# illini-robomaster/irmv_detection

Hardware: AMD Instinct MI355X
Metric: end-to-end FPS (preprocess→NMS→PnP) 640×640 YOLOv8n, 1/2/4/8 MI355X (higher is better)
Workload: dtype f16

## Files before the change

### irmv_detection_amd/csrc/irmv_common.hpp

```cpp
#pragma once

#include <hip/hip_runtime.h>

#include <cstdint>
#include <cstdlib>

namespace irmv {

typedef _Float16 half_t;
typedef _Float16 half8 __attribute__((ext_vector_type(8)));
typedef _Float16 half4 __attribute__((ext_vector_type(4)));
typedef float f32x4 __attribute__((ext_vector_type(4)));

constexpr float kActScale = 1.44269504088896341f;
constexpr float kActUnscale = 0.693147180559945309f;
typedef unsigned int u32x4_t __attribute__((ext_vector_type(4)));
__device__ __forceinline__ float silu_rcp(float y) { return __builtin_amdgcn_rcpf(1.0f + __builtin_amdgcn_exp2f(-y)); }
__device__ __forceinline__ unsigned int silu_pack2(float y0, float y1)
{
    const float r0 = silu_rcp(y0), r1 = silu_rcp(y1);
    unsigned int o;
    asm("v_fma_mixlo_f16 %0, %1, %2, 0" : "=v"(o) : "v"(y0), "v"(r0));
    asm("v_fma_mixhi_f16 %0, %1, %2, 0" : "+v"(o) : "v"(y1), "v"(r1));
    return o;
}
__device__ __forceinline__ half8 silu_pack8(float y0, float y1, float y2, float y3, float y4, float y5, float y6, float y7)
{
    return __builtin_bit_cast(half8, (u32x4_t){silu_pack2(y0, y1), silu_pack2(y2, y3), silu_pack2(y4, y5), silu_pack2(y6, y7)});
}
__device__ __forceinline__ half4 silu_pack4(float y0, float y1, float y2, float y3)
{
    typedef unsigned int u32x2_t __attribute__((ext_vector_type(2)));
    return __builtin_bit_cast(half4, (u32x2_t){silu_pack2(y0, y1), silu_pack2(y2, y3)});
}
__device__ __forceinline__ void mfma_operand_fence(half4 &x) { asm volatile("s_nop 1" : "+v"(x)); }
__device__ __forceinline__ void mfma_operand_fence(half8 &x, half8 &y) { asm volatile("s_nop 1" : "+v"(x), "+v"(y)); }
__device__ __forceinline__ half_t silu_add_res(float y, float res)
{
    float p = y * silu_rcp(y);
    asm("" : "+v"(p));
    float s = p + res;
    asm("" : "+v"(s));
    return (half_t)s;
}

__device__ __forceinline__ void tile_image(int id, int tiles, int batch, int xcd, int &tile, int &image)
{
    const int full = xcd ? (batch >> 3) * 8 * tiles : 0;
    if (id < full) {
        const int j = id >> 3;
        image = (j / tiles) * 8 + (id & 7);
        tile = j % tiles;
    } else {
        const int r = id - full;
        image = (full / tiles) + r / tiles;
        tile = r % tiles;
    }
}

inline int xcd_image_order()
{
    const char *v = getenv("IRMV_XCD_IMAGES");
    return (v && v[0] == '0') ? 0 : 1;
}

inline int wres_stagger()
{
    const char *v = getenv("IRMV_WRES_STAGGER");
    return (v && v[0] == '0') ? 0 : 1;
}

constexpr int kHeadRec = 96;
constexpr int kClsOff = 64;
constexpr int kKptOff = 80;
constexpr int kCandCap = 8192;
constexpr int kMaxDetCap = 256;

struct AxisTap { int32_t i0, i1, w1, pad; };

struct PreArgs {
    const uint8_t *src;
    half_t *dst;
    const AxisTap *tx, *ty;
    int sw, sh, net, swap_rb;
    size_t src_slot_bytes;
};
void launch_preprocess(const PreArgs &a, int batch, hipStream_t s);
void launch_rotate180(const uint8_t *src, uint8_t *dst, int sw, int sh, hipStream_t s);
void launch_upload_frames(const uint8_t *src_host_mapped, uint8_t *dst, size_t bytes, int blocks, hipStream_t s);

constexpr int kBayerBandRows = 8;
struct BayerArgs {
    const uint8_t *raw;
    uint8_t *dst;
    size_t raw_slot_bytes, dst_slot_bytes;
    int W, H;
    int ry, rx;
    uint32_t gain[3];
};
void launch_demosaic(const BayerArgs &a, int batch, hipStream_t s);

struct Conv0Args {
    const half_t *x;
    half_t *y;
    const half_t *w;
    const float *b;
    int net, batch;
};
void launch_conv0(const Conv0Args &a, hipStream_t s);

constexpr int kFrontTileY = 4, kFrontTileX = 16;
constexpr int kFrontTileYDirect = 8;
constexpr int kFrontStageMax = 128 * 1024;
struct FrontArgs {
    const uint8_t *src;
    size_t src_slot_bytes;
    const AxisTap *tx, *ty;
    int vx0, vx1, vy0, vy1;
    int sw, sh, net, swap_rb;
    int fastx, fx_i0, fx_step;
    const half_t *w0;
    const float *b0;
    const half_t *w1;
    const float *b1;
    half_t *out;
    int out_ld;
    int tiles_x, tiles_y;
    int tile_y;
    int stage_bytes;
};
int front_min_stage_bytes(int tile_y = kFrontTileY);
bool front_prepare();
bool launch_front(const FrontArgs &a, int batch, hipStream_t s);

constexpr int kC2fTile = 16;
struct C2fArgs {
    const half_t *x;
    int x_ld;
    half_t *out;
    int out_ld;
    int S, tiles;
    const half_t *w_cv1, *w_m1, *w_m2, *w_cv2;
    const float *b_cv1, *b_m1, *b_m2, *b_cv2;
};
void launch_c2f2(const C2fArgs &a, int batch, hipStream_t s);

struct DwArgs {
    const half_t *x;
    int x_ld;
    half_t *y;
    int y_ld;
    const half_t *w;
    const float *b;
    int Hin, Win, Hout, Wout, C, stride;
};
void launch_dwconv3x3(const DwArgs &a, int batch, hipStream_t s);
struct ShufArgs {
    const half_t *a, *b;
    int a_ld, b_ld;
    half_t *out;
    int out_ld, bc;
    size_t pixels;
};
void launch_shuffle_cat(const ShufArgs &a, hipStream_t s);

struct ConvSeg {
    const half_t *p;
    int ld;
    int C;
    int shift;
};

constexpr int kC2f32TileH = 8, kC2f32TileW = 16;
struct C2f32Args {
    ConvSeg s0, s1;
    int cin1;
    half_t *cat;
    int cat_ld, prev_coff;
    half_t *out;
    int out_ld;
    int H, W, tiles_x, tiles_y;
    const half_t *w_cv1, *w_m1, *w_m2, *w_cv2;
    const float *b_cv1, *b_m1, *b_m2, *b_cv2;
};
size_t c2f32_lds_bytes(int mode);
bool launch_c2f32(int mode, bool shortcut, const C2f32Args &a, int batch, hipStream_t s);

constexpr int kBneckTile = 8;
struct BneckArgs {
    const half_t *yin;
    int yin_ld;
    half_t *ynext;
    int ynext_ld;
    const half_t *cat;
    int cat_ld;
    half_t *out;
    int out_ld;
    int H, W, tiles_x, tiles_y;
    const half_t *w_m1, *w_m2;
    const float *b_m1, *b_m2;
    const half_t *w_cv2;
    const float *b_cv2;
};
size_t bneck64_lds_bytes(int mode, int ks2);
bool launch_bneck64(int mode, int ks2, bool shortcut, const BneckArgs &a, int batch, hipStream_t s);

constexpr int kKpt3Tile = 10;
struct Kpt3Args {
    const half_t *x;
    int x_ld;
    int H, W, tiles_x, tiles_y;
    const half_t *w1;
    const float *b1;
    const half_t *w2;
    const float *b2;
    const half_t *w3;
    const float *b3;
    float *out;
    int out_ld;
};
bool kpt3_eligible(int cin);
bool launch_kpt3(const Kpt3Args &a, int cin, int batch, hipStream_t s);

struct ConvArgs {
    ConvSeg s0, s1;
    int Hin, Win;
    int Hout, Wout;
    int M;
    int Cin;
    const half_t *w;
    const float *bias;
    void *out;
    int out_ld;
    const half_t *res;
    int res_ld;
    int cout_pad;
    int ksteps;
    int pair;
    const half_t *w2;
    const float *bias2;
    float *out2;
    int out2_ld, n2;
    unsigned long long *scan_keys;
    int *scan_counts;
    float scan_thr;
    int scan_nc, scan_abase, scan_key_cap;
};

constexpr int kMultiMax = 6;
struct LdsMember {
    ConvArgs a;
    const half_t *wl;
    int tiles_x, tiles_y, twc_log2, patch_bytes, batch, tile2d;
    int gx, gy;
};
struct LdsMultiArgs {
    int n;
    int start[kMultiMax + 1];
    LdsMember m[kMultiMax];
};
struct DirectMultiArgs {
    int n;
    int start[kMultiMax + 1], gx[kMultiMax], gy[kMultiMax];
    ConvArgs a[kMultiMax];
};

struct ConvCfg {
    int ks, stride, mt, nt; bool cin16; int act; bool out_f32; bool lds; int ipw;
    bool deep;
    bool ct;
    bool pw;
    bool pf2;
    bool pf4;
    bool w8;
    int cm;
    bool wr;
    bool pp;
};
bool launch_conv(const ConvCfg &cfg, const ConvArgs &a, hipStream_t s);
const char *conv_cfg_name(const ConvCfg &cfg, char *buf, int n);
bool conv_pw_eligible(const ConvCfg &cfg, const ConvArgs &a);
bool launch_conv_lds_multi(int nt, const ConvArgs *a, const half_t *const *wl, int n, int batch, hipStream_t s);
bool launch_conv_direct_multi(const ConvCfg &cfg, const ConvArgs *a, int n, hipStream_t s);
bool launch_conv_k16(const ConvArgs &a, hipStream_t s);
bool launch_conv_pw(const ConvCfg &cfg, const ConvArgs &a, hipStream_t s);
size_t conv_pw_lds_bytes(const ConvArgs &a, int nbw);
size_t conv_lds_bytes(const ConvArgs &a, int stride, int mt, int nt, int *patch_rows_max, bool w8 = false);
size_t conv_wres_bytes(const ConvArgs &a, int stride, bool pp);
int conv_wres_tiles(const ConvArgs &a, int stride, bool pp);
bool launch_conv_wres(int ipw, const ConvArgs &a, const half_t *wl, int batch, hipStream_t s, bool pp);
bool launch_conv_lds(int stride, int mt, int nt, int ipw, const ConvArgs &a, const half_t *wl, int batch, hipStream_t s, int pf2 = 0, int cm = 0, bool w8 = false);

void launch_sppf_pool(half_t *buf, int batch, int H, int W, int C, hipStream_t s);

struct DevDet {
    float box_net[4];
    float xyxy[4];
    float score;
    int32_t cls, anchor, pnp_ok;
    float kpts_net[8];
    float kpts[8];
    double rvec[3], tvec[3], quat[4];
    int32_t armor_valid;
    int32_t armor_size;
    int32_t n_lights;
    int32_t pad_;
};
struct DevFrameOut { int32_t num_dets, n_candidates, overflow, pad; };

struct PnpConst {
    double fx, fy, cx, cy, k1, k2, p1, p2, k3;
    double hy[2], hz[2];
};

struct PostArgs {
    const float *head_all;
    int slots_total, first;
    float *boxes;
    unsigned long long *keys;
    int key_cap;
    DevDet *dets;
    DevFrameOut *fout;
    int net, A, nc, nk;
    float logit_thr, iou_thr;
    int max_det, pre_nms_cap;
    float scale_x, scale_y, off_x, off_y;
    int armor_size;
    const PnpConst *pnp;
    long long *dbg;
    int keys_only;
    int prefilter;
    int classwalk;
    int *counts;
};
void launch_nms_pnp(const PostArgs &a, int batch, hipStream_t s);
constexpr int kScanBlocks = 16;
void launch_scan_decode(const PostArgs &a, int batch, hipStream_t s);
constexpr int kLightLdsPoints = 256;
constexpr int kLightLdsImage = 40 * 1024;
constexpr int kLightMaxContours = 1024;

struct LightArgs {
    const uint8_t *frames;
    size_t frame_bytes;
    int cols, rows, rotate180;
    DevDet *dets;
    int max_det;
    const int *num_dets;
    int num_dets_stride, n_boxes;
    const float *boxes;
    signed char *labels;
    size_t label_pool;
    short *points;
    int points_cap;
    short *hulls;
    int binary_threshold;
    float light_min_ratio, light_max_ratio, light_max_angle;
    double min_small_cd, max_small_cd, min_large_cd, max_large_cd;
    const PnpConst *pnp;
    int pnp_armor_size;
};
void launch_light_extract(const LightArgs &a, int n_boxes_max, int batch, hipStream_t s);

void launch_pnp_only(const PnpConst &c, const float *pts, int n, int armor_size, double *rvec, double *tvec,
                     int32_t *ok, hipStream_t s);

}
```

### irmv_detection_amd/csrc/k_c2f.hip

```cpp
#include "irmv_common.hpp"

#include <cstdlib>
#include <mutex>

namespace irmv {

namespace {
constexpr int T = kC2fTile;
constexpr int XW = T + 4, XN = XW * XW;
constexpr int TW = T + 2, TN = TW * TW;
constexpr int HP = 32;

__device__ __forceinline__ f32x4 bias4(const float *b) { return (f32x4){b[0], b[1], b[2], b[3]}; }

typedef unsigned int u32x4 __attribute__((ext_vector_type(4)));
__device__ __forceinline__ u32x4 ld16(const half_t *p) { return *reinterpret_cast<const u32x4 *>(p); }
__device__ __forceinline__ u32x4 keep_if(bool c, u32x4 v) { return c ? v : (u32x4){0u, 0u, 0u, 0u}; }
__device__ __forceinline__ half8 as_h8(u32x4 v) { return __builtin_bit_cast(half8, v); }

template <int RH, int RW>
__device__ __forceinline__ bool region_tile_px(int t, int r, int &ly, int &lx)
{
    constexpr int LC = RW - 16;
    static_assert(LC == 2 || LC == 4, "16 columns + a power of two");
    if (t < RH) { ly = t; lx = r; return true; }
    const int q = (t - RH) * 16 + r;
    const bool ok = q < LC * RH;
    ly = ok ? q / LC : 0;
    lx = ok ? 16 + (q & (LC - 1)) : 0;
    return ok;
}
}

__global__ __launch_bounds__(256) void c2f2_kernel(C2fArgs a, int batch, int xcd)
{
    __shared__ __attribute__((aligned(16))) uint8_t s_y0[T * T * HP];
    __shared__ __attribute__((aligned(16))) uint8_t s_y1[XN * HP];
    __shared__ __attribute__((aligned(16))) uint8_t s_t[TN * HP];
    __shared__ __attribute__((aligned(16))) uint8_t s_y2[T * T * HP];
    const int tid = threadIdx.x, lane = tid & 63, wave = tid >> 6;
    const int g = lane >> 4, r = lane & 15;
    int tile_id, b;
    tile_image(blockIdx.x, a.tiles * a.tiles, batch, xcd, tile_id, b);
    const int tyi = tile_id / a.tiles, txi = tile_id - tyi * a.tiles;
    const int oy0 = tyi * T, ox0 = txi * T;
    const int S = a.S;
    const half8 zero8 = (half8){0, 0, 0, 0, 0, 0, 0, 0};

    const half8 *w;
    w = reinterpret_cast<const half8 *>(a.w_cv1) + lane;
    const half8 Wc1[2] = {w[0], w[64]};
    half8 Wm1[5], Wm2[5];
    w = reinterpret_cast<const half8 *>(a.w_m1) + lane;
#pragma unroll
    for (int ks = 0; ks < 5; ks++) Wm1[ks] = w[ks * 64];
    float bias_c1[8];
#pragma unroll
    for (int i = 0; i < 8; i++) bias_c1[i] = a.b_cv1[g * 8 + i];
    __shared__ float s_bias[16 + 16 + 32];
    if (tid < 16) { s_bias[tid] = a.b_m1[tid]; s_bias[16 + tid] = a.b_m2[tid]; }
    else if (tid < 48) s_bias[16 + tid] = a.b_cv2[tid - 16];

    {
        const float (&bias)[8] = bias_c1;
        constexpr int NROWT = XW / 4, NCOLT = (XN / 16 - XW + 3) / 4;
        static_assert(XW % 4 == 0 && XW - 16 == 4 && NCOLT == 2, "20 row tiles + 5 column tiles");
        const char *xbase = reinterpret_cast<const char *>(a.x);
        const uint32_t img = (uint32_t)b * (uint32_t)(S * S);
        auto px_off = [&](int gy, int gx) -> uint32_t {
            const int gyc = gy < 0 ? 0 : (gy >= S ? S - 1 : gy), gxc = gx < 0 ? 0 : (gx >= S ? S - 1 : gx);
            return ((img + (uint32_t)(gyc * S + gxc)) * (uint32_t)a.x_ld + 8u * g) * 2u;
        };
        const int gx_r = ox0 - 2 + r;
        const bool in_x = (unsigned)gx_r < (unsigned)S;
        int ly_c[NCOLT], lx_c[NCOLT];
        bool has_c[NCOLT];
#pragma unroll
        for (int k = 0; k < NCOLT; k++) {
            const int tc = wave + 4 * k, q = tc * 16 + r;
            has_c[k] = tc < XN / 16 - XW;
            ly_c[k] = has_c[k] ? q >> 2 : 0;
            lx_c[k] = 16 + (q & 3);
        }
        u32x4 Bq[NROWT + NCOLT];
#pragma unroll
        for (int i = 0; i < NROWT; i++) Bq[i] = *reinterpret_cast<const u32x4 *>(xbase + px_off(oy0 - 2 + wave + 4 * i, gx_r));
#pragma unroll
        for (int k = 0; k < NCOLT; k++) Bq[NROWT + k] = *reinterpret_cast<const u32x4 *>(xbase + px_off(oy0 - 2 + ly_c[k], ox0 - 2 + lx_c[k]));
        auto run_tile = [&](u32x4 bq, int ly, int lx, bool inside) {
            const int m = ly * XW + lx;
            f32x4 acc0 = bias4(bias), acc1 = bias4(bias + 4);
            acc0 = __builtin_amdgcn_mfma_f32_16x16x32_f16(Wc1[0], as_h8(bq), acc0, 0, 0, 0);
            acc1 = __builtin_amdgcn_mfma_f32_16x16x32_f16(Wc1[1], as_h8(bq), acc1, 0, 0, 0);
            half8 o = zero8;
            if (inside) o = silu_pack8(acc0[0], acc0[1], acc0[2], acc0[3], acc1[0], acc1[1], acc1[2], acc1[3]);
            if (g >= 2) {
                *reinterpret_cast<half8 *>(s_y1 + m * HP + (g - 2) * 16) = o;
            } else if ((unsigned)(ly - 2) < (unsigned)T && (unsigned)(lx - 2) < (unsigned)T) {
                *reinterpret_cast<half8 *>(s_y0 + ((ly - 2) * T + (lx - 2)) * HP + g * 16) = o;
            }
        };
#pragma unroll
        for (int i = 0; i < NROWT; i++) {
            const int t = wave + 4 * i, gy = oy0 - 2 + t;
            run_tile(Bq[i], t, r, in_x && (unsigned)gy < (unsigned)S);
        }
#pragma unroll
        for (int k = 0; k < NCOLT; k++) {
            if (!has_c[k]) break;
            const int gy = oy0 - 2 + ly_c[k], gx = ox0 - 2 + lx_c[k];
            run_tile(Bq[NROWT + k], ly_c[k], lx_c[k], (unsigned)gy < (unsigned)S && (unsigned)gx < (unsigned)S);
        }
    }
    __syncthreads();

    w = reinterpret_cast<const half8 *>(a.w_m2) + lane;
#pragma unroll
    for (int ks = 0; ks < 5; ks++) Wm2[ks] = w[ks * 64];
    w = reinterpret_cast<const half8 *>(a.w_cv2) + lane;
    const half8 Wc2[2][2] = {{w[0], w[64]}, {w[128], w[192]}};

    {
        float bias[4];
#pragma unroll
        for (int i = 0; i < 4; i++) bias[i] = s_bias[g * 4 + i];
        int toff[5];
#pragma unroll
        for (int ks = 0; ks < 5; ks++) {
            const int tap = 2 * ks + (g >> 1), kh = tap / 3, kw = tap - kh * 3;
            toff[ks] = tap < 9 ? (kh * XW + kw) * HP + 16 * (g & 1) : -1;
        }
        for (int t = wave; t < (TN + 15) / 16; t += 4) {
            int ly, lx;
            const bool mv = region_tile_px<TW, TW>(t, r, ly, lx);
            const int m = ly * TW + lx;
            const uint8_t *base = s_y1 + (ly * XW + lx) * HP;
            f32x4 acc = bias4(bias);
#pragma unroll
            for (int ks = 0; ks < 5; ks++) {
                half8 B = zero8;
                if (toff[ks] >= 0) B = *reinterpret_cast<const half8 *>(base + toff[ks]);
                acc = __builtin_amdgcn_mfma_f32_16x16x32_f16(Wm1[ks], B, acc, 0, 0, 0);
            }
            if (mv) {
                const int gy = oy0 - 1 + ly, gx = ox0 - 1 + lx;
                half4 o = (half4){0, 0, 0, 0};
                if ((unsigned)gy < (unsigned)S && (unsigned)gx < (unsigned)S) o = silu_pack4(acc[0], acc[1], acc[2], acc[3]);
                *reinterpret_cast<half4 *>(s_t + m * HP + g * 8) = o;
            }
        }
    }
    __syncthreads();

    {
        float bias[4];
#pragma unroll
        for (int i = 0; i < 4; i++) bias[i] = s_bias[16 + g * 4 + i];
        int toff[5];
#pragma unroll
        for (int ks = 0; ks < 5; ks++) {
            const int tap = 2 * ks + (g >> 1), kh = tap / 3, kw = tap - kh * 3;
            toff[ks] = tap < 9 ? (kh * TW + kw) * HP + 16 * (g & 1) : -1;
        }
        for (int t = wave; t < T * T / 16; t += 4) {
            const int m = t * 16 + r;
            const int ly = m / T, lx = m - ly * T;
            const uint8_t *base = s_t + (ly * TW + lx) * HP;
            f32x4 acc = bias4(bias);
#pragma unroll
            for (int ks = 0; ks < 5; ks++) {
                half8 B = zero8;
                if (toff[ks] >= 0) B = *reinterpret_cast<const half8 *>(base + toff[ks]);
                acc = __builtin_amdgcn_mfma_f32_16x16x32_f16(Wm2[ks], B, acc, 0, 0, 0);
            }
            const half4 rv = *reinterpret_cast<const half4 *>(s_y1 + ((ly + 2) * XW + lx + 2) * HP + g * 8);
            half4 o;
#pragma unroll
            for (int i = 0; i < 4; i++) o[i] = silu_add_res(acc[i], (float)rv[i]);
            *reinterpret_cast<half4 *>(s_y2 + m * HP + g * 8) = o;
        }
    }
    __syncthreads();

    {
        float bias[8];
#pragma unroll
        for (int i = 0; i < 8; i++) bias[i] = s_bias[32 + g * 8 + i];
        half_t *out = a.out + (size_t)b * S * S * a.out_ld;
        for (int t = wave; t < T * T / 16; t += 4) {
            const int m = t * 16 + r;
            const int ly = m / T, lx = m - ly * T;
            const half8 B0 = g < 2 ? *reinterpret_cast<const half8 *>(s_y0 + m * HP + g * 16)
                                   : *reinterpret_cast<const half8 *>(s_y1 + ((ly + 2) * XW + lx + 2) * HP + (g - 2) * 16);
            half8 B1 = zero8;
            if (g < 2) B1 = *reinterpret_cast<const half8 *>(s_y2 + m * HP + g * 16);
            f32x4 acc0 = bias4(bias), acc1 = bias4(bias + 4);
            acc0 = __builtin_amdgcn_mfma_f32_16x16x32_f16(Wc2[0][0], B0, acc0, 0, 0, 0);
            acc1 = __builtin_amdgcn_mfma_f32_16x16x32_f16(Wc2[1][0], B0, acc1, 0, 0, 0);
            acc0 = __builtin_amdgcn_mfma_f32_16x16x32_f16(Wc2[0][1], B1, acc0, 0, 0, 0);
            acc1 = __builtin_amdgcn_mfma_f32_16x16x32_f16(Wc2[1][1], B1, acc1, 0, 0, 0);
            const int gy = oy0 + ly, gx = ox0 + lx;
            if (gy < S && gx < S) {
                const half8 o = silu_pack8(acc0[0], acc0[1], acc0[2], acc0[3], acc1[0], acc1[1], acc1[2], acc1[3]);
                *reinterpret_cast<half8 *>(out + ((size_t)gy * S + gx) * a.out_ld + g * 8) = o;
            }
        }
    }
}

static int c2f_xcd_order() { return xcd_image_order(); }

void launch_c2f2(const C2fArgs &a, int batch, hipStream_t s)
{
    hipLaunchKernelGGL(c2f2_kernel, dim3(a.tiles * a.tiles * batch), dim3(256), 0, s, a, batch, c2f_xcd_order());
}


namespace {
constexpr int FH = kC2f32TileH, FW = kC2f32TileW;
constexpr int R1H = FH + 4, R1W = FW + 4, R1N = R1H * R1W;
constexpr int R2H = FH + 2, R2W = FW + 2, R2N = R2H * R2W;
constexpr int R3N = FH * FW;
constexpr int PS = 96;
static_assert(R1N % 16 == 0 && R3N % 16 == 0, "tile regions are whole MFMA tiles");
}

template <int MODE, int KS1, bool SHORTCUT>
__global__ __launch_bounds__(256) void c2f32_kernel(C2f32Args a, int batch, int xcd)
{
    extern __shared__ __attribute__((aligned(16))) uint8_t smem[];
    uint8_t *s_in = smem;
    uint8_t *s_t = s_in + R1N * PS;
    uint8_t *s_yn = s_t + R2N * PS;
    uint8_t *s_y0 = s_yn + R3N * PS;
    const int tid = threadIdx.x, lane = tid & 63, wave = tid >> 6;
    const int g = lane >> 4, r = lane & 15;
    int tile_id, b;
    tile_image(blockIdx.x, a.tiles_x * a.tiles_y, batch, xcd, tile_id, b);
    const int tyi = tile_id / a.tiles_x, txi = tile_id - tyi * a.tiles_x;
    const int oy0 = tyi * FH, ox0 = txi * FW;
    const int H = a.H, W = a.W;
    const half8 zero8 = (half8){0, 0, 0, 0, 0, 0, 0, 0};
    half_t *cat = a.cat + (size_t)b * H * W * a.cat_ld;
    __shared__ float s_bias[32 + 32 + 64];
    if (tid < 32) { s_bias[tid] = a.b_m1[tid]; s_bias[32 + tid] = a.b_m2[tid]; }
    if (MODE != 1 && tid < 64) s_bias[64 + tid] = a.b_cv2[tid];

    u32x4 Y01[2][2];
    static_assert(R3N / 16 == 8, "two output tiles per wave");
    if constexpr (MODE != 2) {
        half8 W1[4][KS1];
        {
            const half8 *w = reinterpret_cast<const half8 *>(a.w_cv1) + lane;
#pragma unroll
            for (int nt = 0; nt < 4; nt++)
#pragma unroll
                for (int ks = 0; ks < KS1; ks++) W1[nt][ks] = w[(size_t)(nt * KS1 + ks) * 64];
        }
        float bias[16];
#pragma unroll
        for (int u = 0; u < 2; u++)
#pragma unroll
            for (int i = 0; i < 8; i++) bias[u * 8 + i] = a.b_cv1[u * 32 + g * 8 + i];
        const int H0 = H >> a.s0.shift, W0 = W >> a.s0.shift, H1 = H >> a.s1.shift, W1s = W >> a.s1.shift;
        constexpr int NT1 = R1N / 16, NROWT = R1H / 4, NCOLT = NT1 - R1H;
        static_assert(R1H % 4 == 0 && NCOLT >= 0 && NCOLT <= 4 && R1W - 16 == 4, "three row tiles per wave, at most one column tile");
        const char *base0 = reinterpret_cast<const char *>(a.s0.p), *base1 = reinterpret_cast<const char *>(a.s1.p - a.s0.C);
        const uint32_t img0 = (uint32_t)b * (uint32_t)(H0 * W0), img1 = (uint32_t)b * (uint32_t)(H1 * W1s);
        auto px_off = [&](int gyc, int gxc, uint32_t &o0, uint32_t &o1) {
            o0 = ((img0 + (uint32_t)((gyc >> a.s0.shift) * W0 + (gxc >> a.s0.shift))) * (uint32_t)a.s0.ld + 8u * g) * 2u;
            o1 = ((img1 + (uint32_t)((gyc >> a.s1.shift) * W1s + (gxc >> a.s1.shift))) * (uint32_t)a.s1.ld + 8u * g) * 2u;
        };
        auto issue = [&](uint32_t o0, uint32_t o1, u32x4 (&B)[KS1]) {
#pragma unroll
            for (int ks = 0; ks < KS1; ks++) {
                const bool seg0 = ks * 32 < a.s0.C;
                B[ks] = *reinterpret_cast<const u32x4 *>((seg0 ? base0 : base1) + ((seg0 ? o0 : o1) + (uint32_t)(ks * 64)));
            }
        };
        const int gx_r = ox0 - 2 + r;
        const bool in_x = (unsigned)gx_r < (unsigned)W;
        const int gxc_r = gx_r < 0 ? 0 : (gx_r >= W ? W - 1 : gx_r);
        auto row_off = [&](int t, uint32_t &o0, uint32_t &o1) {
            const int gy = oy0 - 2 + t, gyc = gy < 0 ? 0 : (gy >= H ? H - 1 : gy);
            px_off(gyc, gxc_r, o0, o1);
        };
        const int q_c = 16 * wave + r, ly_c = q_c >> 2, lx_c = 16 + (q_c & 3);
        const bool has_col = wave < NCOLT;
        auto run_tile = [&](const u32x4 (&Bq)[KS1], int ly, int lx, bool inside, bool want_y0) {
            const int m = ly * R1W + lx;
            const int gy = oy0 - 2 + ly, gx = ox0 - 2 + lx;
            f32x4 acc[4];
#pragma unroll
            for (int nt = 0; nt < 4; nt++) acc[nt] = bias4(bias + (nt >> 1) * 8 + (nt & 1) * 4);
            if (want_y0) {
#pragma unroll
                for (int ks = 0; ks < KS1; ks++)
#pragma unroll
                    for (int nt = 0; nt < 4; nt++) acc[nt] = __builtin_amdgcn_mfma_f32_16x16x32_f16(W1[nt][ks], as_h8(Bq[ks]), acc[nt], 0, 0, 0);
            } else {
#pragma unroll
                for (int ks = 0; ks < KS1; ks++)
#pragma unroll
                    for (int nt = 2; nt < 4; nt++) acc[nt] = __builtin_amdgcn_mfma_f32_16x16x32_f16(W1[nt][ks], as_h8(Bq[ks]), acc[nt], 0, 0, 0);
            }
            half8 o[2];
#pragma unroll
            for (int u = 0; u < 2; u++) {
                o[u] = zero8;
                if (inside && (u == 1 || want_y0)) {
                    o[u] = silu_pack8(acc[2 * u][0], acc[2 * u][1], acc[2 * u][2], acc[2 * u][3], acc[2 * u + 1][0], acc[2 * u + 1][1], acc[2 * u + 1][2], acc[2 * u + 1][3]);
                }
            }
            *reinterpret_cast<half8 *>(s_in + m * PS + g * 16) = o[1];
            const int cy = ly - 2, cx = lx - 2;
            if (inside && (unsigned)cy < (unsigned)FH && (unsigned)cx < (unsigned)FW) {
                if constexpr (MODE == 0) {
                    *reinterpret_cast<half8 *>(s_y0 + (cy * FW + cx) * PS + g * 16) = o[0];
                } else {
                    half_t *qd = cat + ((size_t)gy * W + gx) * a.cat_ld + g * 8;
                    *reinterpret_cast<half8 *>(qd) = o[0];
                    *reinterpret_cast<half8 *>(qd + 32) = o[1];
                }
            }
        };
        u32x4 Bn[KS1], Bc[KS1];
        {
            uint32_t o0, o1;
            row_off(wave, o0, o1);
            issue(o0, o1, Bn);
        }
#pragma unroll
        for (int i = 0; i < NROWT; i++) {
            const int t = wave + 4 * i;
#pragma unroll
            for (int ks = 0; ks < KS1; ks++) Bc[ks] = Bn[ks];
            {
                uint32_t o0, o1;
                if (i + 1 < NROWT) {
                    row_off(t + 4, o0, o1);
                    issue(o0, o1, Bn);
                } else if (has_col) {
                    const int gy = oy0 - 2 + ly_c, gx = ox0 - 2 + lx_c;
                    px_off(gy < 0 ? 0 : (gy >= H ? H - 1 : gy), gx < 0 ? 0 : (gx >= W ? W - 1 : gx), o0, o1);
                    issue(o0, o1, Bn);
                }
            }
            const int gy = oy0 - 2 + t;
            run_tile(Bc, t, r, in_x && (unsigned)gy < (unsigned)H, t >= 2 && t < R1H - 2);
        }
        if (has_col) {
            const int gy = oy0 - 2 + ly_c, gx = ox0 - 2 + lx_c;
            run_tile(Bn, ly_c, lx_c, (unsigned)gy < (unsigned)H && (unsigned)gx < (unsigned)W, true);
        }
    } else {
#pragma unroll
        for (int i = 0; i < 2; i++) {
            const int m = (wave + 4 * i) * 16 + r;
            const int ly = m / FW, lx = m - ly * FW;
            const int gy = oy0 + ly, gx = ox0 + lx;
            const bool in = gy < H && gx < W;
            const half_t *q = cat + ((size_t)(in ? gy : 0) * W + (in ? gx : 0)) * a.cat_ld + g * 8;
            Y01[i][0] = ld16(q);
            Y01[i][1] = ld16(q + 32);
        }
        const half_t *src = cat + a.prev_coff;
        constexpr int NP = (R1N * 4 + 255) / 256;
        u32x4 v[NP];
#pragma unroll
        for (int i = 0; i < NP; i++) {
            const int e = tid + i * 256;
            const int m = e >> 2, q = e & 3;
            const int ly = m / R1W, lx = m - ly * R1W;
            const int gy = oy0 - 2 + ly, gx = ox0 - 2 + lx;
            const bool in = e < R1N * 4 && (unsigned)gy < (unsigned)H && (unsigned)gx < (unsigned)W;
            v[i] = ld16(src + ((size_t)(in ? gy : 0) * W + (in ? gx : 0)) * a.cat_ld + q * 8);
        }
#pragma unroll
        for (int i = 0; i < NP; i++) {
            const int e = tid + i * 256;
            const int m = e >> 2;
            const int ly = m / R1W, lx = m - ly * R1W;
            const int gy = oy0 - 2 + ly, gx = ox0 - 2 + lx;
            if (e < R1N * 4) *reinterpret_cast<u32x4 *>(s_in + m * PS + (e & 3) * 16) = keep_if((unsigned)gy < (unsigned)H && (unsigned)gx < (unsigned)W, v[i]);
        }
    }
    __syncthreads();

    {
        half8 Wm[2][9];
        const half8 *w = reinterpret_cast<const half8 *>(a.w_m1) + lane;
#pragma unroll
        for (int nt = 0; nt < 2; nt++)
#pragma unroll
            for (int tap = 0; tap < 9; tap++) Wm[nt][tap] = w[(size_t)(nt * 9 + tap) * 64];
        float bias[8];
#pragma unroll
        for (int i = 0; i < 8; i++) bias[i] = s_bias[g * 8 + i];
        for (int t = wave; t < (R2N + 15) / 16; t += 4) {
            int ly, lx;
            const bool mv = region_tile_px<R2H, R2W>(t, r, ly, lx);
            const int m = ly * R2W + lx;
            const uint8_t *base = s_in + (ly * R1W + lx) * PS + g * 16;
            f32x4 acc0 = bias4(bias), acc1 = bias4(bias + 4);
#pragma unroll
            for (int tap = 0; tap < 9; tap++) {
                const half8 B = *reinterpret_cast<const half8 *>(base + ((tap / 3) * R1W + (tap % 3)) * PS);
                acc0 = __builtin_amdgcn_mfma_f32_16x16x32_f16(Wm[0][tap], B, acc0, 0, 0, 0);
                acc1 = __builtin_amdgcn_mfma_f32_16x16x32_f16(Wm[1][tap], B, acc1, 0, 0, 0);
            }
            if (mv) {
                const int gy = oy0 - 1 + ly, gx = ox0 - 1 + lx;
                half8 o = zero8;
                if ((unsigned)gy < (unsigned)H && (unsigned)gx < (unsigned)W) o = silu_pack8(acc0[0], acc0[1], acc0[2], acc0[3], acc1[0], acc1[1], acc1[2], acc1[3]);
                *reinterpret_cast<half8 *>(s_t + m * PS + g * 16) = o;
            }
        }
    }
    __syncthreads();

    {
        half8 Wm[2][9];
        const half8 *w = reinterpret_cast<const half8 *>(a.w_m2) + lane;
#pragma unroll
        for (int nt = 0; nt < 2; nt++)
#pragma unroll
            for (int tap = 0; tap < 9; tap++) Wm[nt][tap] = w[(size_t)(nt * 9 + tap) * 64];
        float bias[8];
#pragma unroll
        for (int i = 0; i < 8; i++) bias[i] = s_bias[32 + g * 8 + i];
        for (int t = wave; t < R3N / 16; t += 4) {
            const int m = t * 16 + r;
            const int ly = m / FW, lx = m - ly * FW;
            const uint8_t *base = s_t + (ly * R2W + lx) * PS + g * 16;
            f32x4 acc0 = bias4(bias), acc1 = bias4(bias + 4);
#pragma unroll
            for (int tap = 0; tap < 9; tap++) {
                const half8 B = *reinterpret_cast<const half8 *>(base + ((tap / 3) * R2W + (tap % 3)) * PS);
                acc0 = __builtin_amdgcn_mfma_f32_16x16x32_f16(Wm[0][tap], B, acc0, 0, 0, 0);
                acc1 = __builtin_amdgcn_mfma_f32_16x16x32_f16(Wm[1][tap], B, acc1, 0, 0, 0);
            }
            half8 o;
            half8 rv = zero8;
            if constexpr (SHORTCUT) rv = *reinterpret_cast<const half8 *>(s_in + ((ly + 2) * R1W + lx + 2) * PS + g * 16);
            if constexpr (SHORTCUT) {
#pragma unroll
                for (int i = 0; i < 8; i++) o[i] = silu_add_res(i < 4 ? acc0[i] : acc1[i - 4], (float)rv[i]);
            } else {
                o = silu_pack8(acc0[0], acc0[1], acc0[2], acc0[3], acc1[0], acc1[1], acc1[2], acc1[3]);
            }
            if constexpr (MODE == 1) {
                const int gy = oy0 + ly, gx = ox0 + lx;
                if (gy < H && gx < W) *reinterpret_cast<half8 *>(cat + ((size_t)gy * W + gx) * a.cat_ld + 64 + g * 8) = o;
            } else {
                *reinterpret_cast<half8 *>(s_yn + m * PS + g * 16) = o;
            }
        }
    }
    if constexpr (MODE == 1) return;
    __syncthreads();

    {
        constexpr int KS2 = MODE == 0 ? 3 : 4;
        half8 W2[4][KS2];
        const half8 *w = reinterpret_cast<const half8 *>(a.w_cv2) + lane;
#pragma unroll
        for (int nt = 0; nt < 4; nt++)
#pragma unroll
            for (int ks = 0; ks < KS2; ks++) W2[nt][ks] = w[(size_t)(nt * KS2 + ks) * 64];
        float bias[16];
#pragma unroll
        for (int u = 0; u < 2; u++)
#pragma unroll
            for (int i = 0; i < 8; i++) bias[u * 8 + i] = s_bias[64 + u * 32 + g * 8 + i];
        half_t *out = a.out + (size_t)b * H * W * a.out_ld;
        for (int t = wave; t < R3N / 16; t += 4) {
            const int m = t * 16 + r;
            const int ly = m / FW, lx = m - ly * FW;
            const int gy = oy0 + ly, gx = ox0 + lx;
            const bool inside = gy < H && gx < W;
            half8 B[KS2];
            if constexpr (MODE == 0) {
                B[0] = *reinterpret_cast<const half8 *>(s_y0 + m * PS + g * 16);
                B[1] = *reinterpret_cast<const half8 *>(s_in + ((ly + 2) * R1W + lx + 2) * PS + g * 16);
                B[2] = *reinterpret_cast<const half8 *>(s_yn + m * PS + g * 16);
            } else {
                B[0] = as_h8(keep_if(inside, Y01[(t - wave) >> 2][0]));
                B[1] = as_h8(keep_if(inside, Y01[(t - wave) >> 2][1]));
                B[2] = *reinterpret_cast<const half8 *>(s_in + ((ly + 2) * R1W + lx + 2) * PS + g * 16);
                B[3] = *reinterpret_cast<const half8 *>(s_yn + m * PS + g * 16);
            }
            f32x4 acc[4];
#pragma unroll
            for (int nt = 0; nt < 4; nt++) acc[nt] = bias4(bias + (nt >> 1) * 8 + (nt & 1) * 4);
#pragma unroll
            for (int ks = 0; ks < KS2; ks++)
#pragma unroll
                for (int nt = 0; nt < 4; nt++) acc[nt] = __builtin_amdgcn_mfma_f32_16x16x32_f16(W2[nt][ks], B[ks], acc[nt], 0, 0, 0);
            if (inside) {
#pragma unroll
                for (int u = 0; u < 2; u++) {
                    const half8 o = silu_pack8(acc[2 * u][0], acc[2 * u][1], acc[2 * u][2], acc[2 * u][3], acc[2 * u + 1][0], acc[2 * u + 1][1], acc[2 * u + 1][2], acc[2 * u + 1][3]);
                    *reinterpret_cast<half8 *>(out + ((size_t)gy * W + gx) * a.out_ld + u * 32 + g * 8) = o;
                }
            }
        }
    }
}

static std::mutex g_c2f_attr_mu;

size_t c2f32_lds_bytes(int mode) { return (size_t)(R1N + R2N + (mode == 1 ? 0 : R3N) + (mode == 0 ? R3N : 0)) * PS; }

bool launch_c2f32(int mode, bool shortcut, const C2f32Args &a, int batch, hipStream_t s)
{
    const int ks1 = a.cin1 / 32;
    const dim3 grid(a.tiles_x * a.tiles_y * batch), block(256);
    const int xcd = c2f_xcd_order();
    const size_t lds = c2f32_lds_bytes(mode);
#define IRMV_C2F32(MODE_, KS_, SC_)                                                                               \
    if (mode == MODE_ && (MODE_ == 2 || ks1 == KS_) && shortcut == SC_) {                                          \
        static unsigned long long attr_done = 0;                                                                   \
        int dev = 0; (void)hipGetDevice(&dev);                                                                     \
        {                                    \
            std::lock_guard<std::mutex> lk(g_c2f_attr_mu);                                                         \
            if (!(attr_done & (1ull << (dev & 63)))) {                                                             \
                (void)hipFuncSetAttribute(reinterpret_cast<const void *>(c2f32_kernel<MODE_, KS_, SC_>), hipFuncAttributeMaxDynamicSharedMemorySize, 96 * 1024); \
                attr_done |= 1ull << (dev & 63);                                                                   \
            }                                                                                                      \
        }                                                                                                          \
        hipLaunchKernelGGL((c2f32_kernel<MODE_, KS_, SC_>), grid, block, lds, s, a, batch, xcd);                   \
        return true;                                                                                               \
    }
    IRMV_C2F32(0, 2, true) IRMV_C2F32(0, 2, false) IRMV_C2F32(0, 4, false) IRMV_C2F32(0, 6, false) IRMV_C2F32(0, 6, true) IRMV_C2F32(0, 4, true)
    IRMV_C2F32(1, 2, true) IRMV_C2F32(1, 2, false) IRMV_C2F32(1, 4, true) IRMV_C2F32(1, 6, true)
    IRMV_C2F32(2, 1, true) IRMV_C2F32(2, 1, false)
#undef IRMV_C2F32
    return false;
}

}
```

Measured before the change: 61900.

## Shrink c2f32 LDS pixel stride with XOR swizzle and stage cv1 weights in LDS

Reduces the per-pixel LDS stride from 96 to 64 bytes and adds an XOR slot swizzle so MFMA operand reads avoid bank conflicts. Tap and row addresses are now precomputed and advanced incrementally. In mode 0 the cv1 weights are staged through LDS, reusing the buffer later taken by the intermediate tiles, which frees registers. The LDS buffers are reordered so more workgroups fit per CU (static asserts target 3-4 per CU). The trade is extra LDS traffic for the weights in mode 0 and an added barrier.

```diff
diff --git a/irmv_detection_amd/csrc/irmv_common.hpp b/irmv_detection_amd/csrc/irmv_common.hpp
--- a/irmv_detection_amd/csrc/irmv_common.hpp
+++ b/irmv_detection_amd/csrc/irmv_common.hpp
@@ -183,7 +183,7 @@
     const half_t *w_cv1, *w_m1, *w_m2, *w_cv2;
     const float *b_cv1, *b_m1, *b_m2, *b_cv2;
 };
-size_t c2f32_lds_bytes(int mode);
+size_t c2f32_lds_bytes(int mode, int ks1);
 bool launch_c2f32(int mode, bool shortcut, const C2f32Args &a, int batch, hipStream_t s);
 
 constexpr int kBneckTile = 8;
diff --git a/irmv_detection_amd/csrc/k_c2f.hip b/irmv_detection_amd/csrc/k_c2f.hip
--- a/irmv_detection_amd/csrc/k_c2f.hip
+++ b/irmv_detection_amd/csrc/k_c2f.hip
@@ -221,8 +221,40 @@
 constexpr int R1H = FH + 4, R1W = FW + 4, R1N = R1H * R1W;
 constexpr int R2H = FH + 2, R2W = FW + 2, R2N = R2H * R2W;
 constexpr int R3N = FH * FW;
-constexpr int PS = 96;
+constexpr int PS = 64;
 static_assert(R1N % 16 == 0 && R3N % 16 == 0, "tile regions are whole MFMA tiles");
+static_assert(R1W % 2 == 0 && R2W % 2 == 0, "px_addr's slot pattern repeats every 8 pixels: even row widths keep tap shifts and tile steps on it");
+
+__device__ __forceinline__ int px_addr(int p, int g) { return p * PS + (((g ^ (p >> 1)) & 3) << 4); }
+template <int RW> constexpr int rows4() { static_assert((4 * RW) % 8 == 0, "four rows are whole slot periods"); return 4 * RW * PS; }
+template <int D> __device__ __forceinline__ int px_next(int a)
+{
+    static_assert(D % 4 == 0, "the slot moves by 0 or 2");
+    return (D % 8 ? a ^ 32 : a) + D * PS;
+}
+template <int RW> __device__ __forceinline__ void tap_addrs(int p, int g, int (&a)[9])
+{
+#pragma unroll
+    for (int kw = 0; kw < 3; kw++) {
+        a[kw] = px_addr(p + kw, g);
+        if constexpr (RW % 4 == 0) a[3 + kw] = px_next<RW>(a[kw]);
+        else a[3 + kw] = px_addr(p + RW + kw, g);
+        a[6 + kw] = px_next<2 * RW>(a[kw]);
+    }
+}
+
+constexpr int c2f32_w1_bytes(int ks1) { return 4 * ks1 * 1024; }
+constexpr size_t c2f32_lds(int mode, int ks1)
+{
+    return mode == 0 ? (size_t)(R1N + R3N) * PS + (size_t)((R2N + R3N) * PS > c2f32_w1_bytes(ks1) ? (R2N + R3N) * PS : c2f32_w1_bytes(ks1))
+                     : (size_t)(R1N + R2N + (mode == 2 ? R3N : 0)) * PS;
+}
+constexpr size_t kC2f32StaticLds = 512;
+constexpr size_t kCuLds = 160 * 1024;
+constexpr int kC2f32WgPerCu[3] = {3, 4, 4};
+static_assert(kC2f32WgPerCu[0] * (c2f32_lds(0, 6) + kC2f32StaticLds) <= kCuLds, "mode AB: 3 workgroups per CU");
+static_assert(kC2f32WgPerCu[1] * (c2f32_lds(1, 6) + kC2f32StaticLds) <= kCuLds, "mode A: 4 workgroups per CU");
+static_assert(kC2f32WgPerCu[2] * (c2f32_lds(2, 1) + kC2f32StaticLds) <= kCuLds, "mode B: 4 workgroups per CU");
 }
 
 template <int MODE, int KS1, bool SHORTCUT>
@@ -230,9 +262,10 @@
 {
     extern __shared__ __attribute__((aligned(16))) uint8_t smem[];
     uint8_t *s_in = smem;
-    uint8_t *s_t = s_in + R1N * PS;
+    uint8_t *s_y0 = s_in + R1N * PS;
+    uint8_t *s_t = s_y0 + (MODE == 0 ? R3N * PS : 0);
     uint8_t *s_yn = s_t + R2N * PS;
-    uint8_t *s_y0 = s_yn + R3N * PS;
+    uint8_t *s_w1 = s_t;
     const int tid = threadIdx.x, lane = tid & 63, wave = tid >> 6;
     const int g = lane >> 4, r = lane & 15;
     int tile_id, b;
@@ -249,14 +282,23 @@
     u32x4 Y01[2][2];
     static_assert(R3N / 16 == 8, "two output tiles per wave");
     if constexpr (MODE != 2) {
-        half8 W1[4][KS1];
-        {
+        half8 W1[4][MODE == 0 ? 1 : KS1];
+        u32x4 w1_stage[MODE == 0 ? KS1 : 1];
+        if constexpr (MODE == 0) {
+            const u32x4 *w = reinterpret_cast<const u32x4 *>(a.w_cv1) + tid;
+#pragma unroll
+            for (int i = 0; i < KS1; i++) w1_stage[i] = w[i * 256];
+        } else {
             const half8 *w = reinterpret_cast<const half8 *>(a.w_cv1) + lane;
 #pragma unroll
             for (int nt = 0; nt < 4; nt++)
 #pragma unroll
                 for (int ks = 0; ks < KS1; ks++) W1[nt][ks] = w[(size_t)(nt * KS1 + ks) * 64];
         }
+        auto w1 = [&](int nt, int ks) -> half8 {
+            if constexpr (MODE == 0) return *reinterpret_cast<const half8 *>(s_w1 + ((nt * KS1 + ks) * 64 + lane) * 16);
+            else return W1[nt][ks];
+        };
         float bias[16];
 #pragma unroll
         for (int u = 0; u < 2; u++)
@@ -287,8 +329,7 @@
         };
         const int q_c = 16 * wave + r, ly_c = q_c >> 2, lx_c = 16 + (q_c & 3);
         const bool has_col = wave < NCOLT;
-        auto run_tile = [&](const u32x4 (&Bq)[KS1], int ly, int lx, bool inside, bool want_y0) {
-            const int m = ly * R1W + lx;
+        auto run_tile = [&](const u32x4 (&Bq)[KS1], int ly, int lx, bool inside, bool want_y0, int a_y1, int a_y0) {
             const int gy = oy0 - 2 + ly, gx = ox0 - 2 + lx;
             f32x4 acc[4];
 #pragma unroll
@@ -297,12 +338,12 @@
 #pragma unroll
                 for (int ks = 0; ks < KS1; ks++)
 #pragma unroll
-                    for (int nt = 0; nt < 4; nt++) acc[nt] = __builtin_amdgcn_mfma_f32_16x16x32_f16(W1[nt][ks], as_h8(Bq[ks]), acc[nt], 0, 0, 0);
+                    for (int nt = 0; nt < 4; nt++) acc[nt] = __builtin_amdgcn_mfma_f32_16x16x32_f16(w1(nt, ks), as_h8(Bq[ks]), acc[nt], 0, 0, 0);
             } else {
 #pragma unroll
                 for (int ks = 0; ks < KS1; ks++)
 #pragma unroll
-                    for (int nt = 2; nt < 4; nt++) acc[nt] = __builtin_amdgcn_mfma_f32_16x16x32_f16(W1[nt][ks], as_h8(Bq[ks]), acc[nt], 0, 0, 0);
+                    for (int nt = 2; nt < 4; nt++) acc[nt] = __builtin_amdgcn_mfma_f32_16x16x32_f16(w1(nt, ks), as_h8(Bq[ks]), acc[nt], 0, 0, 0);
             }
             half8 o[2];
 #pragma unroll
@@ -312,11 +353,11 @@
                     o[u] = silu_pack8(acc[2 * u][0], acc[2 * u][1], acc[2 * u][2], acc[2 * u][3], acc[2 * u + 1][0], acc[2 * u + 1][1], acc[2 * u + 1][2], acc[2 * u + 1][3]);
                 }
             }
-            *reinterpret_cast<half8 *>(s_in + m * PS + g * 16) = o[1];
+            *reinterpret_cast<half8 *>(s_in + a_y1) = o[1];
             const int cy = ly - 2, cx = lx - 2;
             if (inside && (unsigned)cy < (unsigned)FH && (unsigned)cx < (unsigned)FW) {
                 if constexpr (MODE == 0) {
-                    *reinterpret_cast<half8 *>(s_y0 + (cy * FW + cx) * PS + g * 16) = o[0];
+                    *reinterpret_cast<half8 *>(s_y0 + a_y0) = o[0];
                 } else {
                     half_t *qd = cat + ((size_t)gy * W + gx) * a.cat_ld + g * 8;
                     *reinterpret_cast<half8 *>(qd) = o[0];
@@ -324,11 +365,17 @@
                 }
             }
         };
+        const int a_y1r = px_addr(wave * R1W + r, g), a_y0r = px_addr((wave - 2) * FW + r - 2, g);
         u32x4 Bn[KS1], Bc[KS1];
         {
             uint32_t o0, o1;
             row_off(wave, o0, o1);
             issue(o0, o1, Bn);
+        }
+        if constexpr (MODE == 0) {
+#pragma unroll
+            for (int i = 0; i < KS1; i++) *reinterpret_cast<u32x4 *>(s_w1 + (tid + i * 256) * 16) = w1_stage[i];
+            __syncthreads();
         }
 #pragma unroll
         for (int i = 0; i < NROWT; i++) {
@@ -347,13 +394,122 @@
                 }
             }
             const int gy = oy0 - 2 + t;
-            run_tile(Bc, t, r, in_x && (unsigned)gy < (unsigned)H, t >= 2 && t < R1H - 2);
+            run_tile(Bc, t, r, in_x && (unsigned)gy < (unsigned)H, t >= 2 && t < R1H - 2, a_y1r + i * rows4<R1W>(), a_y0r + i * rows4<FW>());
         }
         if (has_col) {
             const int gy = oy0 - 2 + ly_c, gx = ox0 - 2 + lx_c;
-            run_tile(Bn, ly_c, lx_c, (unsigned)gy < (unsigned)H && (unsigned)gx < (unsigned)W, true);
+            run_tile(Bn, ly_c, lx_c, (unsigned)gy < (unsigned)H && (unsigned)gx < (unsigned)W, true, px_addr(ly_c * R1W + lx_c, g), px_addr((ly_c - 2) * FW + lx_c - 2, g));
         }
     } else {
+        const half_t *src = cat + a.prev_coff;
+        constexpr int NP = (R1N * 4 + 255) / 256;
+        u32x4 v[NP];
+#pragma unroll
+        for (int i = 0; i < NP; i++) {
+            const int e = tid + i * 256;
+            const int m = e >> 2, q = e & 3;
+            const int ly = m / R1W, lx = m - ly * R1W;
+            const int gy = oy0 - 2 + ly, gx = ox0 - 2 + lx;
+            const bool in = e < R1N * 4 && (unsigned)gy < (unsigned)H && (unsigned)gx < (unsigned)W;
+            v[i] = ld16(src + ((size_t)(in ? gy : 0) * W + (in ? gx : 0)) * a.cat_ld + q * 8);
+        }
+#pragma unroll
+        for (int i = 0; i < NP; i++) {
+            const int e = tid + i * 256;
+            const int m = e >> 2;
+            const int ly = m / R1W, lx = m - ly * R1W;
+            const int gy = oy0 - 2 + ly, gx = ox0 - 2 + lx;
+            if (e < R1N * 4) *reinterpret_cast<u32x4 *>(s_in + px_addr(tid >> 2, tid & 3) + i * 64 * PS) = keep_if((unsigned)gy < (unsigned)H && (unsigned)gx < (unsigned)W, v[i]);
+        }
+    }
+    __syncthreads();
+
+    {
+        half8 Wm[2][9];
+        const half8 *w = reinterpret_cast<const half8 *>(a.w_m1) + lane;
+#pragma unroll
+        for (int nt = 0; nt < 2; nt++)
+#pragma unroll
+            for (int tap = 0; tap < 9; tap++) Wm[nt][tap] = w[(size_t)(nt * 9 + tap) * 64];
+        float bias[8];
+#pragma unroll
+        for (int i = 0; i < 8; i++) bias[i] = s_bias[g * 8 + i];
+        int a_in[9];
+        tap_addrs<R1W>(wave * R1W + r, g, a_in);
+        int a_out = px_addr(wave * R2W + r, g);
+        for (int t = wave; t < (R2N + 15) / 16; t += 4) {
+            int ly, lx;
+            const bool mv = region_tile_px<R2H, R2W>(t, r, ly, lx);
+            if (t >= R2H) {
+                tap_addrs<R1W>(ly * R1W + lx, g, a_in);
+                a_out = px_addr(ly * R2W + lx, g);
+            }
+            f32x4 acc0 = bias4(bias), acc1 = bias4(bias + 4);
+#pragma unroll
+            for (int tap = 0; tap < 9; tap++) {
+                const half8 B = *reinterpret_cast<const half8 *>(s_in + a_in[tap]);
+                acc0 = __builtin_amdgcn_mfma_f32_16x16x32_f16(Wm[0][tap], B, acc0, 0, 0, 0);
+                acc1 = __builtin_amdgcn_mfma_f32_16x16x32_f16(Wm[1][tap], B, acc1, 0, 0, 0);
+            }
+            if (mv) {
+                const int gy = oy0 - 1 + ly, gx = ox0 - 1 + lx;
+                half8 o = zero8;
+                if ((unsigned)gy < (unsigned)H && (unsigned)gx < (unsigned)W) o = silu_pack8(acc0[0], acc0[1], acc0[2], acc0[3], acc1[0], acc1[1], acc1[2], acc1[3]);
+                *reinterpret_cast<half8 *>(s_t + a_out) = o;
+            }
+#pragma unroll
+            for (int tap = 0; tap < 9; tap++) a_in[tap] += rows4<R1W>();
+            a_out += rows4<R2W>();
+        }
+    }
+    __syncthreads();
+
+    {
+        half8 Wm[2][9];
+        const half8 *w = reinterpret_cast<const half8 *>(a.w_m2) + lane;
+#pragma unroll
+        for (int nt = 0; nt < 2; nt++)
+#pragma unroll
+            for (int tap = 0; tap < 9; tap++) Wm[nt][tap] = w[(size_t)(nt * 9 + tap) * 64];
+        float bias[8];
+#pragma unroll
+        for (int i = 0; i < 8; i++) bias[i] = s_bias[32 + g * 8 + i];
+        static_assert(FW == 16, "output tile t is row t");
+        int a_in[9];
+        tap_addrs<R2W>(wave * R2W + r, g, a_in);
+        int a_sc = px_addr((wave + 2) * R1W + r + 2, g), a_out = px_addr(wave * FW + r, g);
+        for (int ly = wave; ly < FH; ly += 4) {
+            const int lx = r;
+            f32x4 acc0 = bias4(bias), acc1 = bias4(bias + 4);
+#pragma unroll
+            for (int tap = 0; tap < 9; tap++) {
+                const half8 B = *reinterpret_cast<const half8 *>(s_t + a_in[tap]);
+                acc0 = __builtin_amdgcn_mfma_f32_16x16x32_f16(Wm[0][tap], B, acc0, 0, 0, 0);
+                acc1 = __builtin_amdgcn_mfma_f32_16x16x32_f16(Wm[1][tap], B, acc1, 0, 0, 0);
+            }
+            half8 o;
+            half8 rv = zero8;
+            if constexpr (SHORTCUT) rv = *reinterpret_cast<const half8 *>(s_in + a_sc);
+            if constexpr (SHORTCUT) {
+#pragma unroll
+                for (int i = 0; i < 8; i++) o[i] = silu_add_res(i < 4 ? acc0[i] : acc1[i - 4], (float)rv[i]);
+            } else {
+                o = silu_pack8(acc0[0], acc0[1], acc0[2], acc0[3], acc1[0], acc1[1], acc1[2], acc1[3]);
+            }
+            if constexpr (MODE == 1) {
+                const int gy = oy0 + ly, gx = ox0 + lx;
+                if (gy < H && gx < W) *reinterpret_cast<half8 *>(cat + ((size_t)gy * W + gx) * a.cat_ld + 64 + g * 8) = o;
+            } else {
+                *reinterpret_cast<half8 *>(s_yn + a_out) = o;
+            }
+#pragma unroll
+            for (int tap = 0; tap < 9; tap++) a_in[tap] += rows4<R2W>();
+            a_sc += rows4<R1W>();
+            a_out += rows4<FW>();
+        }
+    }
+    if constexpr (MODE == 1) return;
+    if constexpr (MODE == 2) {
 #pragma unroll
         for (int i = 0; i < 2; i++) {
             const int m = (wave + 4 * i) * 16 + r;
@@ -364,100 +520,7 @@
             Y01[i][0] = ld16(q);
             Y01[i][1] = ld16(q + 32);
         }
-        const half_t *src = cat + a.prev_coff;
-        constexpr int NP = (R1N * 4 + 255) / 256;
-        u32x4 v[NP];
-#pragma unroll
-        for (int i = 0; i < NP; i++) {
-            const int e = tid + i * 256;
-            const int m = e >> 2, q = e & 3;
-            const int ly = m / R1W, lx = m - ly * R1W;
-            const int gy = oy0 - 2 + ly, gx = ox0 - 2 + lx;
-            const bool in = e < R1N * 4 && (unsigned)gy < (unsigned)H && (unsigned)gx < (unsigned)W;
-            v[i] = ld16(src + ((size_t)(in ? gy : 0) * W + (in ? gx : 0)) * a.cat_ld + q * 8);
-        }
-#pragma unroll
-        for (int i = 0; i < NP; i++) {
-            const int e = tid + i * 256;
-            const int m = e >> 2;
-            const int ly = m / R1W, lx = m - ly * R1W;
-            const int gy = oy0 - 2 + ly, gx = ox0 - 2 + lx;
-            if (e < R1N * 4) *reinterpret_cast<u32x4 *>(s_in + m * PS + (e & 3) * 16) = keep_if((unsigned)gy < (unsigned)H && (unsigned)gx < (unsigned)W, v[i]);
-        }
-    }
-    __syncthreads();
-
-    {
-        half8 Wm[2][9];
-        const half8 *w = reinterpret_cast<const half8 *>(a.w_m1) + lane;
-#pragma unroll
-        for (int nt = 0; nt < 2; nt++)
-#pragma unroll
-            for (int tap = 0; tap < 9; tap++) Wm[nt][tap] = w[(size_t)(nt * 9 + tap) * 64];
-        float bias[8];
-#pragma unroll
-        for (int i = 0; i < 8; i++) bias[i] = s_bias[g * 8 + i];
-        for (int t = wave; t < (R2N + 15) / 16; t += 4) {
-            int ly, lx;
-            const bool mv = region_tile_px<R2H, R2W>(t, r, ly, lx);
-            const int m = ly * R2W + lx;
-            const uint8_t *base = s_in + (ly * R1W + lx) * PS + g * 16;
-            f32x4 acc0 = bias4(bias), acc1 = bias4(bias + 4);
-#pragma unroll
-            for (int tap = 0; tap < 9; tap++) {
-                const half8 B = *reinterpret_cast<const half8 *>(base + ((tap / 3) * R1W + (tap % 3)) * PS);
-                acc0 = __builtin_amdgcn_mfma_f32_16x16x32_f16(Wm[0][tap], B, acc0, 0, 0, 0);
-                acc1 = __builtin_amdgcn_mfma_f32_16x16x32_f16(Wm[1][tap], B, acc1, 0, 0, 0);
-            }
-            if (mv) {
-                const int gy = oy0 - 1 + ly, gx = ox0 - 1 + lx;
-                half8 o = zero8;
-                if ((unsigned)gy < (unsigned)H && (unsigned)gx < (unsigned)W) o = silu_pack8(acc0[0], acc0[1], acc0[2], acc0[3], acc1[0], acc1[1], acc1[2], acc1[3]);
-                *reinterpret_cast<half8 *>(s_t + m * PS + g * 16) = o;
-            }
-        }
-    }
-    __syncthreads();
-
-    {
-        half8 Wm[2][9];
-        const half8 *w = reinterpret_cast<const half8 *>(a.w_m2) + lane;
-#pragma unroll
-        for (int nt = 0; nt < 2; nt++)
-#pragma unroll
-            for (int tap = 0; tap < 9; tap++) Wm[nt][tap] = w[(size_t)(nt * 9 + tap) * 64];
-        float bias[8];
-#pragma unroll
-        for (int i = 0; i < 8; i++) bias[i] = s_bias[32 + g * 8 + i];
-        for (int t = wave; t < R3N / 16; t += 4) {
-            const int m = t * 16 + r;
-            const int ly = m / FW, lx = m - ly * FW;
-            const uint8_t *base = s_t + (ly * R2W + lx) * PS + g * 16;
-            f32x4 acc0 = bias4(bias), acc1 = bias4(bias + 4);
-#pragma unroll
-            for (int tap = 0; tap < 9; tap++) {
-                const half8 B = *reinterpret_cast<const half8 *>(base + ((tap / 3) * R2W + (tap % 3)) * PS);
-                acc0 = __builtin_amdgcn_mfma_f32_16x16x32_f16(Wm[0][tap], B, acc0, 0, 0, 0);
-                acc1 = __builtin_amdgcn_mfma_f32_16x16x32_f16(Wm[1][tap], B, acc1, 0, 0, 0);
-            }
-            half8 o;
-            half8 rv = zero8;
-            if constexpr (SHORTCUT) rv = *reinterpret_cast<const half8 *>(s_in + ((ly + 2) * R1W + lx + 2) * PS + g * 16);
-            if constexpr (SHORTCUT) {
-#pragma unroll
-                for (int i = 0; i < 8; i++) o[i] = silu_add_res(i < 4 ? acc0[i] : acc1[i - 4], (float)rv[i]);
-            } else {
-                o = silu_pack8(acc0[0], acc0[1], acc0[2], acc0[3], acc1[0], acc1[1], acc1[2], acc1[3]);
-            }
-            if constexpr (MODE == 1) {
-                const int gy = oy0 + ly, gx = ox0 + lx;
-                if (gy < H && gx < W) *reinterpret_cast<half8 *>(cat + ((size_t)gy * W + gx) * a.cat_ld + 64 + g * 8) = o;
-            } else {
-                *reinterpret_cast<half8 *>(s_yn + m * PS + g * 16) = o;
-            }
-        }
-    }
-    if constexpr (MODE == 1) return;
+    }
     __syncthreads();
 
     {
@@ -468,31 +531,28 @@
         for (int nt = 0; nt < 4; nt++)
 #pragma unroll
             for (int ks = 0; ks < KS2; ks++) W2[nt][ks] = w[(size_t)(nt * KS2 + ks) * 64];
-        float bias[16];
-#pragma unroll
-        for (int u = 0; u < 2; u++)
-#pragma unroll
-            for (int i = 0; i < 8; i++) bias[u * 8 + i] = s_bias[64 + u * 32 + g * 8 + i];
         half_t *out = a.out + (size_t)b * H * W * a.out_ld;
-        for (int t = wave; t < R3N / 16; t += 4) {
-            const int m = t * 16 + r;
-            const int ly = m / FW, lx = m - ly * FW;
+        int a_m = px_addr(wave * FW + r, g), a_y1 = px_addr((wave + 2) * R1W + r + 2, g);
+        for (int i = 0; i < R3N / 16 / 4; i++, a_m += rows4<FW>(), a_y1 += rows4<R1W>()) {
+            const int ly = wave + 4 * i, lx = r;
             const int gy = oy0 + ly, gx = ox0 + lx;
             const bool inside = gy < H && gx < W;
             half8 B[KS2];
             if constexpr (MODE == 0) {
-                B[0] = *reinterpret_cast<const half8 *>(s_y0 + m * PS + g * 16);
-                B[1] = *reinterpret_cast<const half8 *>(s_in + ((ly + 2) * R1W + lx + 2) * PS + g * 16);
-                B[2] = *reinterpret_cast<const half8 *>(s_yn + m * PS + g * 16);
+                B[0] = *reinterpret_cast<const half8 *>(s_y0 + a_m);
+                B[1] = *reinterpret_cast<const half8 *>(s_in + a_y1);
+                B[2] = *reinterpret_cast<const half8 *>(s_yn + a_m);
             } else {
-                B[0] = as_h8(keep_if(inside, Y01[(t - wave) >> 2][0]));
-                B[1] = as_h8(keep_if(inside, Y01[(t - wave) >> 2][1]));
-                B[2] = *reinterpret_cast<const half8 *>(s_in + ((ly + 2) * R1W + lx + 2) * PS + g * 16);
-                B[3] = *reinterpret_cast<const half8 *>(s_yn + m * PS + g * 16);
-            }
+                B[0] = as_h8(keep_if(inside, Y01[i][0]));
+                B[1] = as_h8(keep_if(inside, Y01[i][1]));
+                B[2] = *reinterpret_cast<const half8 *>(s_in + a_y1);
+                B[3] = *reinterpret_cast<const half8 *>(s_yn + a_m);
+            }
+            int boff = 64 + g * 8;
+            asm volatile("" : "+v"(boff));
             f32x4 acc[4];
 #pragma unroll
-            for (int nt = 0; nt < 4; nt++) acc[nt] = bias4(bias + (nt >> 1) * 8 + (nt & 1) * 4);
+            for (int nt = 0; nt < 4; nt++) acc[nt] = bias4(s_bias + boff + (nt >> 1) * 32 + (nt & 1) * 4);
 #pragma unroll
             for (int ks = 0; ks < KS2; ks++)
 #pragma unroll
@@ -510,14 +570,14 @@
 
 static std::mutex g_c2f_attr_mu;
 
-size_t c2f32_lds_bytes(int mode) { return (size_t)(R1N + R2N + (mode == 1 ? 0 : R3N) + (mode == 0 ? R3N : 0)) * PS; }
+size_t c2f32_lds_bytes(int mode, int ks1) { return c2f32_lds(mode, ks1); }
 
 bool launch_c2f32(int mode, bool shortcut, const C2f32Args &a, int batch, hipStream_t s)
 {
     const int ks1 = a.cin1 / 32;
     const dim3 grid(a.tiles_x * a.tiles_y * batch), block(256);
     const int xcd = c2f_xcd_order();
-    const size_t lds = c2f32_lds_bytes(mode);
+    const size_t lds = c2f32_lds_bytes(mode, ks1);
 #define IRMV_C2F32(MODE_, KS_, SC_)                                                                               \
     if (mode == MODE_ && (MODE_ == 2 || ks1 == KS_) && shortcut == SC_) {                                          \
         static unsigned long long attr_done = 0;                                                                   \
```

After: 62280, median of 6. No clear change (+0.6%).
